# smithlabcode/abismal

Hardware: AMD Instinct MI355X
Metric: mapped reads/sec (whole node), 100 bp SE on hg38-scale index (higher is better)
Workload: dtype u64

## Files before the change

abismal_amd/api.py:

```python
import ctypes as C
import os

import numpy as np

_HERE = os.path.dirname(os.path.abspath(__file__))

SE_T_RICH, SE_A_RICH, SE_RANDOM = 0, 1, 2
PE_NORMAL, PE_PBAT, PE_RANDOM = 0, 1, 2
RECORDS_SAM, RECORDS_BAM = 0, 1

HIT_DTYPE = np.dtype([("diffs", "<i2"), ("flags", "<u2"), ("pos", "<u4")])
PAIR_DTYPE = np.dtype([("aln_score", "<i2"), ("reserved", "<i2"), ("r1", HIT_DTYPE), ("r2", HIT_DTYPE)])

EXPORTED_SYMBOLS = [
    "abm_last_error", "abm_default_params", "abm_index_open", "abm_index_close",
    "abm_index_max_candidates", "abm_index_n_chroms", "abm_index_chrom_name",
    "abm_index_chrom_starts", "abm_index_bytes", "abm_index_build", "abm_index_build_targets", "abm_index_build_opts", "abm_index_window", "abm_ctx_create", "abm_ctx_reserve", "abm_ctx_destroy",
    "abm_map_se_batch", "abm_map_se_batch_sliced", "abm_ctx_slice_results", "abm_map_se_device", "abm_map_pe_batch", "abm_map_pe_device",
    "abm_max_read_length", "abm_ctx_reads_too_long", "abm_ctx_filter_on_planes", "abm_ctx_long_cigars", "abm_ctx_take_work", "abm_ctx_set_phase_stamps", "abm_ctx_set_read_cycles", "abm_ctx_set_timing", "abm_ctx_take_kernel_time", "abm_ctx_take_kernel_times", "abm_ctx_take_work_tiers", "abm_stats_allreduce",
    "abm_device_count", "abm_host_alloc", "abm_host_free", "abm_index_set_seed_extension", "abm_index_set_max_candidates", "abm_index_set_direct_narrowing", "abm_ctx_seed_extension", "abm_ctx_rebuild_seed_extension", "abm_device_numa_node",
    "abm_ctx_set_pe_split", "abm_ctx_pe_split_stats", "abm_ctx_pe_timed_launches", "abm_ctx_set_pair_phases", "abm_device_memory", "abm_ctx_pe_footprint", "abm_index_set_seed_extension_cap", "abm_ctx_pinned_bytes", "abm_ctx_set_sam_tails", "abm_ctx_slice_sam_tails", "abm_ctx_pe_sam_tails", "abm_ctx_set_record_format",
    "abm_index_set_window_records", "abm_ctx_window_records",
]


class AbismalAmdError(RuntimeError):
    pass


class Params(C.Structure):
    _fields_ = [("max_candidates", C.c_uint32), ("valid_frac", C.c_double), ("min_frag", C.c_uint32),
                ("max_frag", C.c_uint32), ("allow_ambig", C.c_int32)]

    def __init__(self, max_candidates=0, valid_frac=0.1, min_frag=32, max_frag=3000, allow_ambig=0):
# ... 44 lines not shown
    lib.abm_ctx_destroy.argtypes = [C.c_void_p]
    lib.abm_ctx_reserve.argtypes = [C.c_void_p, C.c_uint64, C.c_uint32, C.c_int]
    lib.abm_max_read_length.restype = C.c_uint32
    lib.abm_ctx_reads_too_long.argtypes = [C.c_void_p]
    lib.abm_ctx_reads_too_long.restype = C.c_uint64
    lib.abm_ctx_filter_on_planes.argtypes = [C.c_void_p]
    lib.abm_ctx_filter_on_planes.restype = C.c_int
    lib.abm_ctx_take_work.argtypes = [C.c_void_p, C.POINTER(C.c_uint64)]
    lib.abm_ctx_long_cigars.argtypes = [C.c_void_p, C.c_void_p, C.c_uint64, C.POINTER(C.c_uint64)]
    lib.abm_ctx_set_timing.argtypes = [C.c_void_p, C.c_int]
    lib.abm_ctx_set_phase_stamps.argtypes = [C.c_void_p, C.c_int]
    lib.abm_ctx_set_read_cycles.argtypes = [C.c_void_p, C.c_void_p]
    lib.abm_ctx_take_kernel_time.argtypes = [C.c_void_p, C.POINTER(C.c_uint64), C.POINTER(C.c_double)]
    lib.abm_ctx_take_kernel_times.argtypes = [C.c_void_p, C.POINTER(C.c_double), C.c_uint64, C.POINTER(C.c_uint64)]
    lib.abm_ctx_take_work_tiers.argtypes = [C.c_void_p, C.POINTER(C.c_uint64)]
    vp = C.c_void_p
    lib.abm_map_se_batch.argtypes = [vp, C.c_int, C.POINTER(Params), C.c_uint64, vp, vp, vp, vp, C.c_uint64, vp]
    lib.abm_map_se_device.argtypes = [vp, C.c_int, C.POINTER(Params), C.c_uint64, vp, vp, C.c_uint32, vp, vp,
                                      C.c_uint32, vp, vp, vp]
    lib.abm_map_pe_batch.argtypes = [vp, C.c_int, C.POINTER(Params), C.c_uint64, vp, vp, vp, vp, vp, vp, vp,
                                     vp, vp, vp, vp, C.c_uint64]
    lib.abm_map_pe_device.argtypes = [vp, C.c_int, C.POINTER(Params), C.c_uint64, vp, vp, vp, vp, C.c_uint32,
                                      vp, vp, vp, vp, vp, C.c_uint32, vp, vp, vp, vp]
    _lib = lib
    return lib


def _check(rc):
    if rc != 0:
        raise AbismalAmdError(load_library().abm_last_error().decode(errors="replace"))
# ... 257 lines not shown
    def take_work_tiers(self):
        out = (C.c_uint64 * 32)()
        _check(self._lib.abm_ctx_take_work_tiers(self.handle, out))
        keys = ["seed_offsets", "search_probes", "candidates", "index_run_lines", "set_updates", "alignments",
                "cyc_probe_narrow", "cyc_gather_hamming", "cyc_replay", "cyc_se_fallback", "cyc_total",
                "window_cache_hits", "cyc_sort_unique", "cyc_score_pairable", "cyc_mate", "cyc_best_single"]
        return [dict(zip(keys, [int(x) for x in out[16 * t:16 * t + 16]])) for t in range(2)]

    def take_work(self):
        out = (C.c_uint64 * 16)()
        _check(self._lib.abm_ctx_take_work(self.handle, out))
        keys = ["seed_offsets", "search_probes", "candidates", "read_words", "set_updates", "alignments"]
        d = dict(zip(keys, [int(x) for x in out[:6]]))
        d["window_cache_hits"] = int(out[11])
        d["single_job_reads"] = int(out[12])
        if out[10]:
            d["light_filter_steps"], d["fifo_updates"], d["filter_steps"] = int(out[13]), int(out[14]), int(out[15])
        if out[10]:
            d["phase_cycles"] = dict(zip(["probe_narrow", "gather_hamming", "replay", "align", "total"],
                                         [int(x) for x in out[6:11]]))
        return d

    def set_pe_split(self, split=-1, seed_cap=0, hand_entries=0):
        self._lib.abm_ctx_set_pe_split.argtypes = [C.c_void_p, C.c_int, C.c_uint32, C.c_uint64]
        _check(self._lib.abm_ctx_set_pe_split(self.handle, int(split), int(seed_cap), int(hand_entries)))

    def pe_split_stats(self):
        out = (C.c_uint64 * 4)()
        self._lib.abm_ctx_pe_split_stats.argtypes = [C.c_void_p, C.POINTER(C.c_uint64)]
        _check(self._lib.abm_ctx_pe_split_stats(self.handle, out))
# ... 18 lines not shown
```

abismal_amd/csrc/abm_api.hip:

```cpp
#include "../../include/abismal_amd.h"
#include "abm_index_file.hpp"
#include "abm_index_build.hpp"
#include "abm_kernels.hpp"

#include <rccl/rccl.h>

#include <algorithm>
#include <cctype>
#include <chrono>
#include <cstdio>
#include <cstdlib>
#include <cstring>
#include <iterator>
#include <map>
#include <mutex>
#include <stdexcept>
#include <string>
#include <thread>
#include <vector>

namespace {

thread_local std::string g_error;

// ... 342 lines not shown
  a.cig_arena_count = ctx->cig_arena_count.p;
  if (pinned) ctx->h_tail.p[0] = ctx->h_tail.p[1] = 0;
  a.cig_arena = pinned ? ctx->h_arena.p : ctx->cig_arena.p;
  a.cig_arena_cap = static_cast<abm::u32>(std::min<size_t>(pinned ? ctx->h_arena.cap : ctx->cig_arena.cap, 0xFFFFFF00u));
}

abm::u32 se_text_stride(const abm_ctx *ctx, const LaunchShape &s, abm::u32 cig_stride, bool host_results, bool sliced) {
  if (!ctx->sam_on || !host_results || !sliced) return 0;
  if (ctx->sam_format == ABM_RECORDS_BAM && ctx->phase_stamps) return 0;
  const abm::u32 stride = ctx->sam_format == ABM_RECORDS_BAM ? bam_stride_for(s.eff_len, cig_stride) : sam_stride_for(ctx, s.eff_len, cig_stride);
  return stride <= abm::sam_line_room(s.GW, s.tb_extra) ? stride : 0;
}

void se_reserve(abm_ctx *ctx, uint64_t n, const LaunchShape &s, uint32_t n_slices, bool host_results, abm::u32 sam_stride) {
  ctx->packed.reserve(n * 4 * s.W); ctx->lens.reserve(n);
  ctx->work.reserve(32); ctx->next_read.reserve(64);
  if (n < (1ull << 32)) {
    ctx->order.reserve(n); ctx->cls.reserve(n);
    if (n_slices) { ctx->slice_id.reserve(n); ctx->slice_left.reserve(n_slices); ctx->slice_hist.reserve(abm::order_sliced_hist_words(n_slices)); }
    else ctx->class33.reserve(33);
  }
  arena_reserve(ctx, 2 * n, host_results);
  if (sam_stride) { ctx->h_sam.reserve(static_cast<size_t>(n) * sam_stride); ctx->h_sam_len.reserve(n); }
}

void se_long_reads(abm_ctx *ctx, const abm::SeArgs &main, uint64_t n, const char *d_blob, const uint64_t *d_off,
                   abm::u32 max_len, double valid_frac, HostMode host, hipStream_t st) {
  if (n >= (1ull << 32)) throw std::invalid_argument("batch too large for the long-read launch (>= 2^32 reads)");
  ctx->long_list.reserve(n);
  ctx->long_count.reserve(1);
  HIPCHK(hipMemsetAsync(ctx->long_count.p, 0, 4, st));
// ... 264 lines not shown
  PeLaunch t2;
};
PePlan pe_plan(const abm_ctx *ctx, uint64_t n, const LaunchShape &s, abm::u32 cig_stride, bool host_results) {
  PePlan p{};
  p.split = pe_split_on(ctx);
  p.sam_stride = pe_text_stride(ctx, s, cig_stride, host_results);
  p.scap = pe_seed_cap(ctx);
  if (p.split) p.seed = pe_seed_launch(s, n);
  else p.t1 = pe_whole_launch(ctx, s, n, false, p.sam_stride != 0);
  p.t2 = pe_whole_launch(ctx, s, n, true, p.sam_stride != 0);
  return p;
}

void pe_reserve(abm_ctx *ctx, uint64_t n, const LaunchShape &s, abm::u32 mode_slots, bool host_results, const PePlan &p) {
  ctx->packed.reserve(n * 4 * s.W); ctx->packed2.reserve(n * 4 * s.W); ctx->lens.reserve(n); ctx->lens2.reserve(n);
  ctx->work.reserve(32); ctx->next_read.reserve(64);
  ctx->order.reserve(n); ctx->cls.reserve(n); ctx->class33.reserve(33);
  ctx->need_big.reserve(n); ctx->subset.reserve(n); ctx->subset_count.reserve(1);
  if (p.sam_stride) { ctx->h_sam.reserve(static_cast<size_t>(2 * n) * p.sam_stride); ctx->h_sam_len.reserve(2 * n); ctx->h_pe_kind.reserve(n); }
  arena_reserve(ctx, 4 * n, host_results);
  if (!p.split) ctx->payload1.reserve(static_cast<size_t>(std::max(p.t1.waves, 0)) * abm::kPeTier1Cap);
  else {
    const size_t hand_cap = pe_hand_entries(ctx, n), stage = p.scap > abm::kPeTier1Cap ? static_cast<size_t>(p.seed.grid) * p.scap : 0;
    ctx->hand_hdr.reserve(n * mode_slots * 2); ctx->hand_count.reserve(1);
    ctx->hand_pos.reserve(hand_cap); ctx->hand_d.reserve(hand_cap);
    ctx->stage_pos.reserve(stage); ctx->stage_d.reserve(stage);
    ctx->subset_b.reserve(n); ctx->subset_count_b.reserve(1); ctx->class33_b.reserve(33);
  }
  pe_tier2_reserve(ctx, static_cast<size_t>(std::max(p.t2.waves, 0)));
}

// ... 479 lines not shown
          rep.dix.wrec = nullptr;
          rep.dix.wrec_t0 = rep.dix.wrec_a0 = rep.dix.wrec_blocks = rep.dix.wrec_back = rep.dix.wrec_max_len = 0;
          try { build_wrec(rep, *ix); build_ext(rep, *ix, tables_maxc); }
          catch (...) { free_wrec(rep); (void)hipFree(arena); rep.arena = nullptr; throw; }
        }
        ++rep.refs;
        c->holds_replica = true;
        c->rep = &rep;
        c->dix = rep.dix;
        c->kernel_turn = &rep.kernel_turn;
      }
      HIPCHK(hipStreamCreateWithFlags(&c->stream, hipStreamNonBlocking));
      HIPCHK(hipEventCreateWithFlags(&c->last_done, hipEventDisableTiming));
      HIPCHK(hipHostMalloc(reinterpret_cast<void **>(&c->drained), sizeof(abm::u32), hipHostMallocMapped | hipHostMallocCoherent));
      *c->drained = 0;
      c->work.reserve(32);
      HIPCHK(hipMemset(c->work.p, 0, 32 * sizeof(unsigned long long)));
    }
    catch (...) { abm_ctx_destroy(c); throw; }
    *out = c;
  });
}

void abm_ctx_destroy(abm_ctx *c) {
  if (!c) return;
  (void)hipSetDevice(c->device);
  if (c->stream) (void)hipStreamDestroy(c->stream);
  if (c->last_done) (void)hipEventDestroy(c->last_done);
  if (c->drained) (void)hipHostFree(c->drained);
  if (c->holds_replica && c->rep) {
    std::lock_guard<std::mutex> lk(c->rep->mu);
    if (--c->rep->refs == 0) {
// ... 38 lines not shown
    unsigned long long tmp[32];
    HIPCHK(hipMemcpy(tmp, ctx->work.p, sizeof(tmp), hipMemcpyDeviceToHost));
    HIPCHK(hipMemset(ctx->work.p, 0, sizeof(tmp)));
    for (int k = 0; k < 16; ++k) out[k] = tmp[k] + tmp[16 + k];
  });
}

int abm_ctx_take_work_tiers(abm_ctx *ctx, uint64_t out[32]) {
  return guarded([&] {
    HIPCHK(hipSetDevice(ctx->device));
    HIPCHK(hipDeviceSynchronize());
    unsigned long long tmp[32];
    HIPCHK(hipMemcpy(tmp, ctx->work.p, sizeof(tmp), hipMemcpyDeviceToHost));
    HIPCHK(hipMemset(ctx->work.p, 0, sizeof(tmp)));
    for (int k = 0; k < 32; ++k) out[k] = tmp[k];
  });
}

int abm_ctx_set_timing(abm_ctx *ctx, int enable) {
  return guarded([&] {
    if (!ctx) throw std::invalid_argument("ctx is null");
    std::lock_guard<std::mutex> lk(ctx->mu);
    ctx->timing = enable != 0;
  });
}

int abm_ctx_take_kernel_time(abm_ctx *ctx, uint64_t *launches, double *total_ms) {
  return guarded([&] {
    if (!ctx || !launches || !total_ms) throw std::invalid_argument("null argument");
    std::lock_guard<std::mutex> lk(ctx->mu);
// ... 393 lines not shown
    std::vector<abm_hit> hits(m), h2(m);
    std::vector<abm_pair> pairs(m);
    std::vector<uint32_t> cig(m * (L + 2)), cig2(m * (L + 2));
    std::vector<uint64_t> co(m + 1), co2(m + 1);
    abm_params par;
    abm_default_params(&par);
    int rc;
    if (!paired) rc = abm_map_se_batch(ctx, ABM_SE_T_RICH, &par, m, blob.data(), off.data(), hits.data(), cig.data(), cig.size(), co.data());
    else rc = abm_map_pe_batch(ctx, ABM_PE_NORMAL, &par, m, blob.data(), off.data(), blob.data(), off.data(), pairs.data(), hits.data(),
                               h2.data(), cig.data(), co.data(), cig2.data(), co2.data(), cig.size());
    if (rc != 0) throw std::runtime_error(g_error);
    {
      std::lock_guard<std::mutex> lk(ctx->mu);
      HIPCHK(hipSetDevice(ctx->device));
      HIPCHK(hipDeviceSynchronize());
      HIPCHK(hipMemset(ctx->work.p, 0, 32 * sizeof(unsigned long long)));
    }
  });
}

int abm_ctx_long_cigars(abm_ctx *ctx, uint32_t *out_ops, uint64_t capacity, uint64_t *n_ops) {
  return guarded([&] {
    if (!ctx || !n_ops) throw std::invalid_argument("null argument");
    std::lock_guard<std::mutex> lk(ctx->mu);
    HIPCHK(hipSetDevice(ctx->device));
    HIPCHK(hipEventSynchronize(ctx->last_done));
    uint32_t cnt = 0;
    if (ctx->cig_arena_count.p) HIPCHK(hipMemcpy(&cnt, ctx->cig_arena_count.p, 4, hipMemcpyDeviceToHost));
    cnt = static_cast<uint32_t>(std::min<uint64_t>(cnt, ctx->cig_arena.cap));
    *n_ops = cnt;
    if (cnt > capacity) throw std::length_error("capacity too small for the long CIGARs");
// ... 66 lines not shown
```

abismal_amd/csrc/abm_kernels.hip:

```cpp
#include <type_traits>
#include "abm_kernels_core.hpp"
#include "abm_sam.hpp"

#ifndef ABM_SE_WAVES_PER_SIMD
#define ABM_SE_WAVES_PER_SIMD 5
#endif


namespace abm {

__global__ __launch_bounds__(256) void pack_reads_kernel(const char *__restrict__ blob,
                                                         const u64 *__restrict__ off, u64 n_reads,
                                                         u32 W, u64 *__restrict__ packed,
                                                         u32 *__restrict__ lens) {
  const u64 gid = static_cast<u64>(blockIdx.x) * blockDim.x + threadIdx.x;
  const u64 r = gid / W;
  const u32 w = static_cast<u32>(gid % W);
  if (r >= n_reads)
    return;
  const u64 b = off[r];
  const u32 L = static_cast<u32>(off[r + 1] - b);
  if (w == 0)
    lens[r] = L;
  u64 ft = 0, fa = 0, rt = 0, ra = 0;
// ... 118 lines not shown
  lds.hres = reinterpret_cast<u16 *>(lds.lbest);
  lds.G = a.G;
  lds.smark[lane] = 0; lds.smark[64 + lane] = 0;
  u32 seg_epoch = 0;

  const u32 n_calls = a.mode == 2 ? 4u : 2u;
  const u32 call_rc = a.mode == 2 ? 0xCu  : 0x2u ;
  const u32 call_ar = a.mode == 2 ? 0x6u  : (a.mode == 1 ? 0x3u : 0x0u);

  WorkTally wt = {0, 0, 0, 0, 0, 0, 0, 0, 0, 0, 0, 0, 0, 0};
  const CigarSink sink = {a.cig_stride, a.ctmp_cap, a.cig_arena, a.cig_arena_count, a.cig_arena_cap, (!LONG && a.sam_tail) ? lds.jpos : nullptr};
  const u64 n_items = a.n_reads;
  long long t_begin = 0, t_a = 0, t_b = 0;
  ABM_STAMP(t_begin);
  u32 n_aln = 0, n_single = 0;
  bool overflow = false, too_long = false;

  const u64 dealt = gridDim.x;
  auto next_read = [&]() -> u64 {
    unsigned long long v = 0;
    if (lane == 0) {
      v = atomicAdd(a.next_read, 1ull) + dealt;
      if (v >= n_items && a.drained) __hip_atomic_store(a.drained, 1u, __ATOMIC_RELAXED, __HIP_MEMORY_SCOPE_SYSTEM);
    }
    return (static_cast<u64>(static_cast<u32>(uni(static_cast<int>(v >> 32)))) << 32) |
           static_cast<u32>(uni(static_cast<int>(v)));
  };
  u64 r_next = blockIdx.x;
  while (r_next < n_items) {
    const u64 slot = r_next;
// ... 28 lines not shown
      SeSet S;
      S.begin_read(L);
      for (u32 cidx = 0; cidx < n_calls; ++cidx) {
        const bool rc = (call_rc >> cidx) & 1u, ar = (call_ar >> cidx) & 1u;
        const bool g_to_a = rc != ar;
        const u32 enc = (rc ? 2u : 0u) + (g_to_a ? 1u : 0u);
        const u32 flags = (rc ? kFlagRC : 0u) | (ar ? kFlagARich : 0u);
        S.cutoff = S.good_cutoff;
        seed_pass<true, TIMED, COOP, REC>(a.ix, lds, enc, g_to_a, flags, L, S, wt, seg_epoch);
        if (S.sz != static_cast<int>(kSeCap) || S.cutoff > S.good_cutoff) {
          S.cutoff = S.top_d();
          seed_pass<false, TIMED, COOP, REC>(a.ix, lds, enc, g_to_a, flags, L, S, wt, seg_epoch);
        }
      }
      ABM_STAMP(t_a);
      choose_se<LONG>(a.ix, lds, L, a.valid_frac, S, best, cig_out, sink, n_ops, rd_overflow, n_aln, n_single);
      overflow |= rd_overflow;
      ABM_STAMP(t_b);
      if (TIMED) wt.t_align += t_b - t_a;
    }
    if constexpr (!LONG) {
      if (a.sam_tail != nullptr) {
        const u32 len = (L > a.max_len) ? 0xFFFFFFFFu : format_sam_tail<BAM>(a, lds.tb, lds.jpos, r, (L >= a.ix.min_len) ? L : 0u, best, best.pos != 0 ? n_ops : 0u);
        if (lane == 0) store_out(a.sam_len + r, len);
      }
    }
    if (lane == 0) {
      store_out(a.res + r, best);
      store_out(a.cig_n + r, best.pos != 0 ? n_ops : 0u);
      if (TIMED && a.read_cycles) a.read_cycles[r] = static_cast<u32>((clock64() - t_read) >> 10);
    }
// ... 19 lines not shown
      atomicAdd(&a.work[2], static_cast<unsigned long long>(s2));
      atomicAdd(&a.work[3], static_cast<unsigned long long>(s3));
      atomicAdd(&a.work[4], static_cast<unsigned long long>(wt.updates));
      atomicAdd(&a.work[5], static_cast<unsigned long long>(n_aln));
      atomicAdd(&a.work[11], static_cast<unsigned long long>(wsum_hits));
      atomicAdd(&a.work[12], static_cast<unsigned long long>(n_single));
      if (TIMED) {
        atomicAdd(&a.work[6], static_cast<unsigned long long>(wt.t_probe));
        atomicAdd(&a.work[7], static_cast<unsigned long long>(wt.t_stream));
        atomicAdd(&a.work[8], static_cast<unsigned long long>(wt.t_replay));
        atomicAdd(&a.work[9], static_cast<unsigned long long>(wt.t_align));
        atomicAdd(&a.work[10], static_cast<unsigned long long>(phase_stamp() - t_begin));
        atomicAdd(&a.work[13], static_cast<unsigned long long>(wt.light_steps));
        atomicAdd(&a.work[14], static_cast<unsigned long long>(wt.fifo_updates));
        atomicAdd(&a.work[15], static_cast<unsigned long long>(wt.steps));
      }
    }
  }
  if (lane == 0 && (overflow || too_long))
    atomicOr(a.status, (overflow ? 1u : 0u) | (too_long ? 2u : 0u));
  if (a.host_tail != nullptr && lane == 0) {
    __threadfence();
    const u32 before = atomicAdd(a.finished, 1u);
    if (before + 1u == gridDim.x) {
      __threadfence();
      a.host_tail[0] = __hip_atomic_load(a.cig_arena_count, __ATOMIC_RELAXED, __HIP_MEMORY_SCOPE_AGENT);
      a.host_tail[1] = __hip_atomic_load(a.status, __ATOMIC_RELAXED, __HIP_MEMORY_SCOPE_AGENT);
    }
  }
}
// ... 364 lines not shown
```

abismal_amd/csrc/abm_kernels.hpp:

```cpp
#pragma once
#include "abm_device.hpp"

namespace abm {

struct SeArgs {
  DevIndex ix;
  const u64 *packed;
  const u32 *lens;
  const u32 *order;
  u64 n_reads;
  u32 W, WB, GW;
  u32 max_len;
  u32 tb_extra;
  u32 G;
  int mode;
  double valid_frac;
  double size_frac;
  Hit *res;
  u32 *cig;
  u32 cig_stride;
  u32 ctmp_cap;
  u8 *long_tb;
  u32 *long_ctmp;
  u64 long_tb_bytes;
// ... 7 lines not shown
  u32 *finished;
  u32 *host_tail;
  const u16 *slice_id;
  u32 *slice_left;
  u32 *slice_done;
  const char *blob;
  const u64 *off;
  char *sam_tail;
  u32 *sam_len;
  u32 sam_stride;
  int sam_allow_ambig;
  int sam_format;
  u32 *read_cycles;
  unsigned long long *work;
};

struct PeArgs {
  DevIndex ix;
  const u64 *packed1, *packed2;
  const u32 *lens1, *lens2;
  const u32 *order;
  const u32 *subset;
  const u32 *subset_count;
  u64 n_pairs;
  u32 W, WB, GW, tb_extra, G, max_len;
  int mode;
  double valid_frac;
  u32 min_frag, max_frag;
  int allow_ambig;
  Hit *pairs;
// ... 105 lines not shown
```

abismal_amd/csrc/abm_kernels_core.hpp:

```cpp
#pragma once
#include "abm_kernels.hpp"

namespace abm {

struct SeSet {
  static constexpr bool kFifo = true;
  static constexpr bool kAppend = false;
  int hk;
  u32 pf;
  u32 pp;
  int sz, cutoff, good_cutoff;
  int best_d;
  u32 best_f, best_p;
  bool sure_ambig;

  __device__ __forceinline__ static int key_d(int k) { return k >> 8; }
  __device__ __forceinline__ void begin_read(u32 readlen) {
    const int worst = static_cast<i16>(0.4 * readlen);
    hk = worst * 256; pf = 0; pp = 0;
    sz = 1;
    cutoff = worst;
    good_cutoff = static_cast<i16>(readlen / 10u);
    best_d = worst; best_f = 0; best_p = 0;
    sure_ambig = false;
// ... 1060 lines not shown
    cur = valid ? c : 0;
    if (valid && c > bestv) { bestv = c; bestrow = i; }
    if (TB && assigned) lds.tb[i * bw + jl] = static_cast<u8>(valid ? (arrow | (c > 0 ? 4 : 0)) : 3);
  }
}

struct CigarSink {
  u32 stride;
  u32 ctmp_cap;
  u32 *arena;
  u32 *arena_count;
  u32 arena_cap;
  u32 *fin;
};

__device__ __forceinline__ void wave_cigar(const u8 *tb, u32 *ctmp, int L, int diffs, int max_diffs,
                                           int score, int best_r, int best_c, u32 *cig_out,
                                           const CigarSink &sink, u32 &n_ops, int &ins, int &del, u32 &aln_len,
                                           u32 &t_pos, bool &overflow) {
  const int lane = lane_id();
  ins = del = 0;
  if (score == 0 || diffs == 0) {
    if (lane == 0) { store_out(cig_out, static_cast<u32>(L) << 4); if (sink.fin) sink.fin[0] = static_cast<u32>(L) << 4; }
    n_ops = 1;
    aln_len = static_cast<u32>(L);
    return;
  }
  const int bw = band_for(diffs, max_diffs);
  int r = best_r, c = best_c;
  const int clip_tail = (L + (bw - 1)) - (r + c);
  u32 n = 0;
  auto emit = [&](u32 run, int op) {
    if (n < sink.ctmp_cap) { if (lane == 0) ctmp[n] = (run << 4) | static_cast<u32>(op); }
    const int r8 = static_cast<int>(static_cast<u8>(run));
    ins = op == 1 ? static_cast<i16>(ins + r8) : ins;
    del = op == 2 ? static_cast<i16>(del + r8) : del;
    ++n;
  };
  auto step = [&](int a) {
    if (a != 1) --r;
    if (a == 1) --c;
    if (a == 2) ++c;
  };
  int op = uni(tb[r * bw + c]) & 3;
  step(op);
  u32 run = 1;
  for (;;) {
    const int cell = uni(tb[r * bw + c]);
    if (!(cell & 4)) break;
    const int a = cell & 3;
    step(a);
    if (a != op) { emit(run, op); run = 0; }
    ++run;
    op = a;
  }
  emit(run, op);
  const int clip_head = (r + c) - (bw - 1);
  wave_sync();
  const u32 full = n + (clip_head > 0) + (clip_tail > 0);
  u32 *dst = cig_out;
  u32 body = n, total = full;
  if (full > sink.stride) {
    u32 at = 0xFFFFFFFFu;
    if (sink.arena != nullptr && n <= sink.ctmp_cap) {
      if (lane == 0) at = atomicAdd(sink.arena_count, full);
      at = static_cast<u32>(uni(static_cast<int>(at)));
      if (at > sink.arena_cap || full > sink.arena_cap - at) at = 0xFFFFFFFFu;
    }
    if (at != 0xFFFFFFFFu) {
      dst = sink.arena + at;
      if (lane == 0) store_out(cig_out, at);
    }
    else {
// ... 1 lines not shown
      body = min(min(n, sink.ctmp_cap), sink.stride);
      total = min(body + (clip_head > 0) + (clip_tail > 0), sink.stride);
    }
  }
  for (u32 k = lane; k < total; k += 64) {
    u32 v;
    const u32 kk = k - (clip_head > 0 ? 1u : 0u);
    if (clip_head > 0 && k == 0) v = (static_cast<u32>(clip_head) << 4) | 4u;
    else if (kk < body) v = ctmp[body - 1 - kk];
    else v = (static_cast<u32>(clip_tail) << 4) | 4u;
    store_out(dst + k, v);
    if (sink.fin && k < kSeCap) sink.fin[k] = v;
  }
  n_ops = full;
  aln_len = static_cast<u32>(L - clip_tail - clip_head);
  t_pos = t_pos - static_cast<u32>((bw - 1) / 2) + static_cast<u32>(r);
}

__device__ __forceinline__ int edit_distance(int scr, u32 len, int ins, int del) {
  if (scr == 0)
    return static_cast<i16>(len);
  const int A = static_cast<i16>(scr + 4 * (ins + del));
  const u32 num = 2u * (len - static_cast<u32>(ins)) - static_cast<u32>(A);
  const int mism = static_cast<i16>(num / 5u);
  return static_cast<i16>(mism + ins + del);
}

__device__ __forceinline__ bool long_enough(u32 aln_len, u32 readlen, u32 kMinReadLen) {
  const double min_frac = 1.0 - 0.4;
  return aln_len >= max(kMinReadLen, static_cast<u32>(min_frac * readlen));
}
// ... 154 lines not shown
}

struct QuadJob {
  u32 mv, ma, ml;
  int qoff_lo, qoff_hi;
  int g_lo, g_hi;
  int gs_lo, gs_hi;
};

typedef unsigned short u16x2 __attribute__((ext_vector_type(2)));
__device__ __forceinline__ int wave_min_i32(int x) {
#pragma unroll
  for (int d = 32; d >= 1; d >>= 1) x = min(x, __shfl_xor(x, d));
  return x;
}
__device__ __forceinline__ void wavefront_quad(const WaveLds &lds, const QuadJob &jp, const QuadJob &jq, int dp, int dq,
                                               int o, int width, int L, int w_min, int w_max, u32 &bestp, u32 &bestq) {
  const int t_start = max(0, w_min - 1), t_end = 2 * (L - 1 + w_max) + 1;
  const int n_total = (t_end - t_start) / 2 + 1;
  const int W = static_cast<int>(lds.W), GW = static_cast<int>(lds.GW);
  const int q0p = ((t_start - dp - o) >> 1) + o - width, q0q = ((t_start + 1 - dq - o) >> 1) + o - width;
  const bool in_slot = width != 0;
  const int q_lo = wave_min_i32(in_slot ? min(q0p, q0q) : 0x3fffffff), q_hi = wave_max_i32(in_slot ? max(q0p, q0q) : -0x3fffffff);
  const int n_mid0 = min(max(1 - q_lo, 0), n_total), n_mid1 = min(max(L - 1 - q_hi, n_mid0), n_total);
  u32 curp = 0, curq = 0, pub = 0, Mp = 0, Mq = 0;
  bestp = bestq = 0;
  auto refill = [&](const QuadJob &j, int q) -> u32 {
    const int i0 = q - o + width;
    u64 lo = 0, hi = 0;
    if (j.mv & 0xFFFFu) lo = nibbles16(lds.qpk + j.qoff_lo, W, q) & nibbles16(lds.gwin + j.g_lo * GW, GW, j.gs_lo + i0 - 1);
    if (j.mv >> 16) hi = nibbles16(lds.qpk + j.qoff_hi, W, q) & nibbles16(lds.gwin + j.g_hi * GW, GW, j.gs_hi + i0 - 1);
    lo |= lo >> 1; lo |= lo >> 2;
    hi |= hi >> 1; hi |= hi >> 2;
    return every_fourth_bit(lo) | (every_fourth_bit(hi) << 16);
  };
  auto step_delta = [&](u32 &M) -> u32 {
    const u16x2 bits = __builtin_bit_cast(u16x2, M & 0x00010001u);
    M >>= 1;
    const u16x2 five = {5, 5}, minus3 = {0xFFFD, 0xFFFD};
    return __builtin_bit_cast(u32, static_cast<u16x2>(bits * five + minus3));
  };
  auto fast = [&](const QuadJob &j, u32 &cur, u32 &M, u32 &best) {
    const u32 lf = static_cast<u32>(from_prev_lane(static_cast<int>(pub))), up = static_cast<u32>(from_next_lane(static_cast<int>(pub)));
    u32 c = pk_max(pk_add(cur, step_delta(M)), 0u);
    c = pk_max(c, pk_add(up, 0xFFFCFFFCu) & j.ma);
    c = pk_max(c, pk_add(lf, 0xFFFCFFFCu) & j.ml);
    cur = c & j.mv;
    best = pk_max(best, cur);
    pub = cur;
  };
  auto slow = [&](const QuadJob &j, int q, u32 &cur, u32 &M, u32 &best) {
    const u32 lf = static_cast<u32>(from_prev_lane(static_cast<int>(pub))), up = static_cast<u32>(from_next_lane(static_cast<int>(pub)));
    u32 c = pk_max(pk_add(cur, step_delta(M)), 0u);
    c = pk_max(c, pk_add(up, 0xFFFCFFFCu) & (q < L - 1 ? j.ma : 0u));
    c = pk_max(c, pk_add(lf, 0xFFFCFFFCu) & (q > 0 ? j.ml : 0u));
    cur = static_cast<u32>(q) < static_cast<u32>(L) ? (c & j.mv) : 0u;
    best = pk_max(best, cur);
    pub = cur;
  };
  int n = 0;
#pragma clang loop unroll(disable)
  for (int seg = 0; seg < 3; ++seg) {
    const int end = seg == 0 ? n_mid0 : (seg == 1 ? n_mid1 : n_total);
    while (n < end) {
      if ((n & 15) == 0) { Mp = refill(jp, n + q0p); Mq = refill(jq, n + q0q); }
      const int stop = min(end, (n | 15) + 1);
      if (seg == 1) {
        for (; n < stop; ++n) { fast(jp, curp, Mp, bestp); fast(jq, curq, Mq, bestq); }
      }
      else {
        for (; n < stop; ++n) { slow(jp, n + q0p, curp, Mp, bestp); slow(jq, n + q0q, curq, Mq, bestq); }
      }
    }
  }
}

__device__ __forceinline__ int score_round_quad(const DevIndex &ix, const WaveLds &lds, int first, int n_jobs, int L, int md,
                                                int qbase) {
  const int lane = lane_id();
  QuadJob ja = {0, 0, 0, 0, 0, 0, 0, 0, 0}, jb = {0, 0, 0, 0, 0, 0, 0, 0, 0};
  int used = 0, s = first, w_min = 64, w_max = 0, my_o = 0, my_w = 0;
  while (s < n_jobs) {
    const int cnt = min(4, n_jobs - s);
    if (s - first + cnt > static_cast<int>(lds.max_jobs)) break;
    int bwh[4], width = 0;
#pragma unroll
    for (int h = 0; h < 4; ++h) {
      bwh[h] = h < cnt ? band_for(static_cast<int>(lds.jdf[s + h]) >> 16, md) : 0;
      width = max(width, bwh[h]);
    }
    if (used + width > 64) break;
    const int o = lane - used, K = (width - 1) / 2, c = o - K;
    const bool in = o >= 0 && o < width;
// ... 14 lines not shown
        const int gs = static_cast<int>(t_beg & 15u) - (K - k);
        if (h >> 1) { j.qoff_hi = qoff; j.g_hi = s + h - first; j.gs_hi = gs; }
        else { j.qoff_lo = qoff; j.g_lo = s + h - first; j.gs_lo = gs; }
      }
    }
    used += width;
    w_min = min(w_min, width);
    w_max = max(w_max, width);
    s += cnt;
  }
  stage_windows(ix, lds, first, s - first, md);
  wave_sync();
  const int t_start = max(0, w_min - 1);
  const bool even = ((t_start - my_o) & 1) == 0;
  u32 bp, bq;
  wavefront_quad(lds, even ? ja : jb, even ? jb : ja, even ? 0 : 1, even ? 1 : 0, my_o, my_w, L, w_min, w_max, bp, bq);
  const u32 best_a = even ? bp : bq, best_b = even ? bq : bp;
  int base = 0, mine = 0;
  for (int k = first; k < s;) {
    const int cnt = min(4, s - k);
    int width = 0;
#pragma unroll
    for (int h = 0; h < 4; ++h)
      if (h < cnt) width = max(width, band_for(static_cast<int>(lds.jdf[k + h]) >> 16, md));
    const bool in = lane >= base && lane < base + width;
    const u32 xa = wave_max_pk(in ? best_a : 0u), xb = cnt > 1 ? wave_max_pk(in ? best_b : 0u) : 0u;
    if (lane == k - first) mine = static_cast<int>(xa & 0xFFFFu);
    if (lane == k + 1 - first && cnt > 1) mine = static_cast<int>(xb & 0xFFFFu);
    if (lane == k + 2 - first && cnt > 2) mine = static_cast<int>(xa >> 16);
    if (lane == k + 3 - first && cnt > 3) mine = static_cast<int>(xb >> 16);
    base += width;
// ... 5 lines not shown
  return s;
}

#ifndef ABM_QUAD_MIN_JOBS
#define ABM_QUAD_MIN_JOBS 1
#endif
constexpr int kQuadMinJobs = ABM_QUAD_MIN_JOBS;
template <bool WRAP = false>
__device__ __forceinline__ int score_jobs(const DevIndex &ix, const WaveLds &lds, int first, int n_jobs, int L, int md, int qbase) {
  if constexpr (!WRAP) {
    if (n_jobs - first >= kQuadMinJobs) return score_round_quad(ix, lds, first, n_jobs, L, md, qbase);
  }
  return score_round<WRAP>(ix, lds, first, n_jobs, L, md, qbase);
}

template <bool WRAP = false>
__device__ __forceinline__ void choose_se(const DevIndex &ix, const WaveLds &lds, u32 L, double frac,
                                          SeSet &S, Hit &best, u32 *cig_out, const CigarSink &sink,
                                          u32 &n_ops, bool &overflow, u32 &n_aln, u32 &n_single) {
  const int lane = lane_id();
  const int Ls = static_cast<i16>(L);
  const int md = static_cast<i16>(frac * static_cast<u32>(Ls));
  const int perfect = static_cast<i16>(2 * L);
  n_ops = 0;
  if (S.best_p != 0) {
    best.diffs = static_cast<i16>(S.best_d); best.flags = static_cast<u16>(S.best_f); best.pos = S.best_p;
    if (lane == 0) { store_out(cig_out, L << 4); if (sink.fin) sink.fin[0] = L << 4; }
    n_ops = 1;
    return;
  }
  const bool mine = lane < S.sz;
  const int slot_of = S.hk & 255;
  const u32 e_pos = __shfl(S.pp, slot_of), e_flags = __shfl(S.pf, slot_of);
  const int e_d = SeSet::key_d(S.hk);
// ... 77 lines not shown
    if (sc <= 0) { best.flags = static_cast<u16>(kFlagAmbig); return; }
  }
  u32 alen = 0, pos = b_pos;
  int n_ins = 0, n_del = 0;
  wave_cigar(lds.tb, lds.ctmp, static_cast<int>(L), b_diffs, md, sc, br, bc, cig_out, sink, n_ops,
             n_ins, n_del, alen, pos, overflow);
  wave_sync();
  const int nm = edit_distance(top, alen, n_ins, n_del);
  if (long_enough(alen, static_cast<u32>(Ls), ix.min_len) && nm <= md) {
    best.diffs = static_cast<i16>(nm);
    best.pos = pos;
  }
}


}
```

include/abismal_amd.h:

```cpp
#ifndef ABISMAL_AMD_H
#define ABISMAL_AMD_H

#include <stddef.h>
#include <stdint.h>

#ifdef __cplusplus
extern "C" {
#endif

typedef struct abm_index abm_index;
typedef struct abm_ctx abm_ctx;

typedef struct { int16_t diffs; uint16_t flags; uint32_t pos; } abm_hit;

typedef struct { int16_t aln_score; int16_t reserved; abm_hit r1, r2; } abm_pair;

typedef struct {
  uint32_t max_candidates;
  double valid_frac;
  uint32_t min_frag;
  uint32_t max_frag;
  int32_t allow_ambig;
} abm_params;

// ... 81 lines not shown
int abm_ctx_long_cigars(abm_ctx *ctx, uint32_t *out_ops, uint64_t capacity, uint64_t *n_ops);

enum {
  ABM_STATUS_CIGAR_OVERFLOW = 1u,
  ABM_STATUS_READ_TOO_LONG = 2u,
  ABM_STATUS_SET_OVERFLOW = 4u
};
uint32_t abm_max_read_length(void);
uint64_t abm_ctx_reads_too_long(abm_ctx *ctx);

int abm_ctx_filter_on_planes(const abm_ctx *ctx);

int abm_ctx_take_work(abm_ctx *ctx, uint64_t out[16]);
int abm_ctx_set_phase_stamps(abm_ctx *ctx, int enable);
int abm_ctx_take_work_tiers(abm_ctx *ctx, uint64_t out[32]);
int abm_ctx_set_read_cycles(abm_ctx *ctx, uint32_t *d_read_cycles);
int abm_ctx_set_pair_phases(abm_ctx *ctx, uint32_t *d_pair_phases);

int abm_ctx_set_timing(abm_ctx *ctx, int enable);
int abm_ctx_take_kernel_time(abm_ctx *ctx, uint64_t *launches, double *total_ms);
int abm_ctx_take_kernel_times(abm_ctx *ctx, double *ms_out, uint64_t capacity, uint64_t *launches);

int abm_stats_allreduce(abm_ctx *const *ctxs, int n_ctx, uint64_t *const *counters);

#ifdef __cplusplus
}
#endif
#endif
```

Before: 22.62 million.

## Score best-diff pilot candidate first and prune remaining wavefronts below its score

For short-read SE mapping, the candidate with the fewest seed diffs is aligned and traced first. Its score then becomes a floor that lets the packed quad wavefront stop early once no lane can reach it, using an upper bound of match score times remaining read bases. If another candidate wins, the traceback is redone for that candidate. The cost is an extra alignment pass in that case, added per-16-step ballot checks, and new iteration counters exposed through the work buffer.

```diff
diff --git a/abismal_amd/api.py b/abismal_amd/api.py
--- a/abismal_amd/api.py
+++ b/abismal_amd/api.py
@@ -17,7 +17,7 @@
     "abm_index_max_candidates", "abm_index_n_chroms", "abm_index_chrom_name",
     "abm_index_chrom_starts", "abm_index_bytes", "abm_index_build", "abm_index_build_targets", "abm_index_build_opts", "abm_index_window", "abm_ctx_create", "abm_ctx_reserve", "abm_ctx_destroy",
     "abm_map_se_batch", "abm_map_se_batch_sliced", "abm_ctx_slice_results", "abm_map_se_device", "abm_map_pe_batch", "abm_map_pe_device",
-    "abm_max_read_length", "abm_ctx_reads_too_long", "abm_ctx_filter_on_planes", "abm_ctx_long_cigars", "abm_ctx_take_work", "abm_ctx_set_phase_stamps", "abm_ctx_set_read_cycles", "abm_ctx_set_timing", "abm_ctx_take_kernel_time", "abm_ctx_take_kernel_times", "abm_ctx_take_work_tiers", "abm_stats_allreduce",
+    "abm_max_read_length", "abm_ctx_reads_too_long", "abm_ctx_filter_on_planes", "abm_ctx_long_cigars", "abm_ctx_take_work", "abm_ctx_set_phase_stamps", "abm_ctx_set_read_cycles", "abm_ctx_set_timing", "abm_ctx_take_kernel_time", "abm_ctx_take_kernel_times", "abm_ctx_take_work_tiers", "abm_ctx_take_score_iterations", "abm_stats_allreduce",
     "abm_device_count", "abm_host_alloc", "abm_host_free", "abm_index_set_seed_extension", "abm_index_set_max_candidates", "abm_index_set_direct_narrowing", "abm_ctx_seed_extension", "abm_ctx_rebuild_seed_extension", "abm_device_numa_node",
     "abm_ctx_set_pe_split", "abm_ctx_pe_split_stats", "abm_ctx_pe_timed_launches", "abm_ctx_set_pair_phases", "abm_device_memory", "abm_ctx_pe_footprint", "abm_index_set_seed_extension_cap", "abm_ctx_pinned_bytes", "abm_ctx_set_sam_tails", "abm_ctx_slice_sam_tails", "abm_ctx_pe_sam_tails", "abm_ctx_set_record_format",
     "abm_index_set_window_records", "abm_ctx_window_records",
@@ -92,6 +92,8 @@
     lib.abm_ctx_take_kernel_time.argtypes = [C.c_void_p, C.POINTER(C.c_uint64), C.POINTER(C.c_double)]
     lib.abm_ctx_take_kernel_times.argtypes = [C.c_void_p, C.POINTER(C.c_double), C.c_uint64, C.POINTER(C.c_uint64)]
     lib.abm_ctx_take_work_tiers.argtypes = [C.c_void_p, C.POINTER(C.c_uint64)]
+    if hasattr(lib, "abm_ctx_take_score_iterations"):
+        lib.abm_ctx_take_score_iterations.argtypes = [C.c_void_p, C.POINTER(C.c_uint64)]
     vp = C.c_void_p
     lib.abm_map_se_batch.argtypes = [vp, C.c_int, C.POINTER(Params), C.c_uint64, vp, vp, vp, vp, C.c_uint64, vp]
     lib.abm_map_se_device.argtypes = [vp, C.c_int, C.POINTER(Params), C.c_uint64, vp, vp, C.c_uint32, vp, vp,
@@ -379,6 +381,10 @@
         d = dict(zip(keys, [int(x) for x in out[:6]]))
         d["window_cache_hits"] = int(out[11])
         d["single_job_reads"] = int(out[12])
+        if out[10] and hasattr(self._lib, "abm_ctx_take_score_iterations"):
+            it = (C.c_uint64 * 2)()
+            _check(self._lib.abm_ctx_take_score_iterations(self.handle, it))
+            d["score_iterations"], d["score_iterations_full"] = int(it[0]), int(it[1])
         if out[10]:
             d["light_filter_steps"], d["fifo_updates"], d["filter_steps"] = int(out[13]), int(out[14]), int(out[15])
         if out[10]:
diff --git a/abismal_amd/csrc/abm_api.hip b/abismal_amd/csrc/abm_api.hip
--- a/abismal_amd/csrc/abm_api.hip
+++ b/abismal_amd/csrc/abm_api.hip
@@ -380,7 +380,7 @@
 
 void se_reserve(abm_ctx *ctx, uint64_t n, const LaunchShape &s, uint32_t n_slices, bool host_results, abm::u32 sam_stride) {
   ctx->packed.reserve(n * 4 * s.W); ctx->lens.reserve(n);
-  ctx->work.reserve(32); ctx->next_read.reserve(64);
+  ctx->work.reserve(abm::kWorkWords); ctx->next_read.reserve(64);
   if (n < (1ull << 32)) {
     ctx->order.reserve(n); ctx->cls.reserve(n);
     if (n_slices) { ctx->slice_id.reserve(n); ctx->slice_left.reserve(n_slices); ctx->slice_hist.reserve(abm::order_sliced_hist_words(n_slices)); }
@@ -675,7 +675,7 @@
 
 void pe_reserve(abm_ctx *ctx, uint64_t n, const LaunchShape &s, abm::u32 mode_slots, bool host_results, const PePlan &p) {
   ctx->packed.reserve(n * 4 * s.W); ctx->packed2.reserve(n * 4 * s.W); ctx->lens.reserve(n); ctx->lens2.reserve(n);
-  ctx->work.reserve(32); ctx->next_read.reserve(64);
+  ctx->work.reserve(abm::kWorkWords); ctx->next_read.reserve(64);
   ctx->order.reserve(n); ctx->cls.reserve(n); ctx->class33.reserve(33);
   ctx->need_big.reserve(n); ctx->subset.reserve(n); ctx->subset_count.reserve(1);
   if (p.sam_stride) { ctx->h_sam.reserve(static_cast<size_t>(2 * n) * p.sam_stride); ctx->h_sam_len.reserve(2 * n); ctx->h_pe_kind.reserve(n); }
@@ -1185,8 +1185,8 @@
       HIPCHK(hipEventCreateWithFlags(&c->last_done, hipEventDisableTiming));
       HIPCHK(hipHostMalloc(reinterpret_cast<void **>(&c->drained), sizeof(abm::u32), hipHostMallocMapped | hipHostMallocCoherent));
       *c->drained = 0;
-      c->work.reserve(32);
-      HIPCHK(hipMemset(c->work.p, 0, 32 * sizeof(unsigned long long)));
+      c->work.reserve(abm::kWorkWords);
+      HIPCHK(hipMemset(c->work.p, 0, abm::kWorkWords * sizeof(unsigned long long)));
     }
     catch (...) { abm_ctx_destroy(c); throw; }
     *out = c;
@@ -1255,6 +1255,18 @@
     HIPCHK(hipMemcpy(tmp, ctx->work.p, sizeof(tmp), hipMemcpyDeviceToHost));
     HIPCHK(hipMemset(ctx->work.p, 0, sizeof(tmp)));
     for (int k = 0; k < 32; ++k) out[k] = tmp[k];
+  });
+}
+
+int abm_ctx_take_score_iterations(abm_ctx *ctx, uint64_t out[2]) {
+  return guarded([&] {
+    if (!ctx) throw std::invalid_argument("ctx is null");
+    HIPCHK(hipSetDevice(ctx->device));
+    HIPCHK(hipDeviceSynchronize());
+    unsigned long long tmp[2];
+    HIPCHK(hipMemcpy(tmp, ctx->work.p + abm::kWorkScoreIters, sizeof(tmp), hipMemcpyDeviceToHost));
+    HIPCHK(hipMemset(ctx->work.p + abm::kWorkScoreIters, 0, sizeof(tmp)));
+    out[0] = tmp[0]; out[1] = tmp[1];
   });
 }
 
@@ -1678,7 +1690,7 @@
       std::lock_guard<std::mutex> lk(ctx->mu);
       HIPCHK(hipSetDevice(ctx->device));
       HIPCHK(hipDeviceSynchronize());
-      HIPCHK(hipMemset(ctx->work.p, 0, 32 * sizeof(unsigned long long)));
+      HIPCHK(hipMemset(ctx->work.p, 0, abm::kWorkWords * sizeof(unsigned long long)));
     }
   });
 }
diff --git a/abismal_amd/csrc/abm_kernels.hip b/abismal_amd/csrc/abm_kernels.hip
--- a/abismal_amd/csrc/abm_kernels.hip
+++ b/abismal_amd/csrc/abm_kernels.hip
@@ -156,6 +156,7 @@
   long long t_begin = 0, t_a = 0, t_b = 0;
   ABM_STAMP(t_begin);
   u32 n_aln = 0, n_single = 0;
+  u32 score_iters[2] = {0, 0};
   bool overflow = false, too_long = false;
 
   const u64 dealt = gridDim.x;
@@ -214,7 +215,7 @@
         }
       }
       ABM_STAMP(t_a);
-      choose_se<LONG>(a.ix, lds, L, a.valid_frac, S, best, cig_out, sink, n_ops, rd_overflow, n_aln, n_single);
+      choose_se<LONG, !LONG, TIMED>(a.ix, lds, L, a.valid_frac, S, best, cig_out, sink, n_ops, rd_overflow, n_aln, n_single, score_iters);
       overflow |= rd_overflow;
       ABM_STAMP(t_b);
       if (TIMED) wt.t_align += t_b - t_a;
@@ -264,6 +265,8 @@
         atomicAdd(&a.work[13], static_cast<unsigned long long>(wt.light_steps));
         atomicAdd(&a.work[14], static_cast<unsigned long long>(wt.fifo_updates));
         atomicAdd(&a.work[15], static_cast<unsigned long long>(wt.steps));
+        atomicAdd(&a.work[kWorkScoreIters], static_cast<unsigned long long>(score_iters[0]));
+        atomicAdd(&a.work[kWorkScoreIters + 1], static_cast<unsigned long long>(score_iters[1]));
       }
     }
   }
diff --git a/abismal_amd/csrc/abm_kernels.hpp b/abismal_amd/csrc/abm_kernels.hpp
--- a/abismal_amd/csrc/abm_kernels.hpp
+++ b/abismal_amd/csrc/abm_kernels.hpp
@@ -45,6 +45,7 @@
   u32 *read_cycles;
   unsigned long long *work;
 };
+constexpr u32 kWorkScoreIters = 32, kWorkWords = 34;
 
 struct PeArgs {
   DevIndex ix;
diff --git a/abismal_amd/csrc/abm_kernels_core.hpp b/abismal_amd/csrc/abm_kernels_core.hpp
--- a/abismal_amd/csrc/abm_kernels_core.hpp
+++ b/abismal_amd/csrc/abm_kernels_core.hpp
@@ -1098,24 +1098,20 @@
   u32 *fin;
 };
 
-__device__ __forceinline__ void wave_cigar(const u8 *tb, u32 *ctmp, int L, int diffs, int max_diffs,
-                                           int score, int best_r, int best_c, u32 *cig_out,
-                                           const CigarSink &sink, u32 &n_ops, int &ins, int &del, u32 &aln_len,
-                                           u32 &t_pos, bool &overflow) {
+struct CigarWalk {
+  u32 n;
+  int clip_head, clip_tail;
+  int r;
+};
+__device__ __forceinline__ CigarWalk cigar_walk(const u8 *tb, u32 *ctmp, u32 ctmp_cap, int L, int bw, int best_r, int best_c,
+                                                int &ins, int &del) {
   const int lane = lane_id();
   ins = del = 0;
-  if (score == 0 || diffs == 0) {
-    if (lane == 0) { store_out(cig_out, static_cast<u32>(L) << 4); if (sink.fin) sink.fin[0] = static_cast<u32>(L) << 4; }
-    n_ops = 1;
-    aln_len = static_cast<u32>(L);
-    return;
-  }
-  const int bw = band_for(diffs, max_diffs);
   int r = best_r, c = best_c;
   const int clip_tail = (L + (bw - 1)) - (r + c);
   u32 n = 0;
   auto emit = [&](u32 run, int op) {
-    if (n < sink.ctmp_cap) { if (lane == 0) ctmp[n] = (run << 4) | static_cast<u32>(op); }
+    if (n < ctmp_cap) { if (lane == 0) ctmp[n] = (run << 4) | static_cast<u32>(op); }
     const int r8 = static_cast<int>(static_cast<u8>(run));
     ins = op == 1 ? static_cast<i16>(ins + r8) : ins;
     del = op == 2 ? static_cast<i16>(del + r8) : del;
@@ -1141,6 +1137,13 @@
   emit(run, op);
   const int clip_head = (r + c) - (bw - 1);
   wave_sync();
+  return {n, clip_head, clip_tail, r};
+}
+__device__ __forceinline__ void cigar_publish(const u32 *ctmp, const CigarWalk &w, int L, int bw, u32 *cig_out,
+                                              const CigarSink &sink, u32 &n_ops, u32 &aln_len, u32 &t_pos, bool &overflow) {
+  const int lane = lane_id();
+  const u32 n = w.n;
+  const int clip_head = w.clip_head, clip_tail = w.clip_tail;
   const u32 full = n + (clip_head > 0) + (clip_tail > 0);
   u32 *dst = cig_out;
   u32 body = n, total = full;
@@ -1172,7 +1175,22 @@
   }
   n_ops = full;
   aln_len = static_cast<u32>(L - clip_tail - clip_head);
-  t_pos = t_pos - static_cast<u32>((bw - 1) / 2) + static_cast<u32>(r);
+  t_pos = t_pos - static_cast<u32>((bw - 1) / 2) + static_cast<u32>(w.r);
+}
+__device__ __forceinline__ void wave_cigar(const u8 *tb, u32 *ctmp, int L, int diffs, int max_diffs,
+                                           int score, int best_r, int best_c, u32 *cig_out,
+                                           const CigarSink &sink, u32 &n_ops, int &ins, int &del, u32 &aln_len,
+                                           u32 &t_pos, bool &overflow) {
+  if (score == 0 || diffs == 0) {
+    ins = del = 0;
+    if (lane_id() == 0) { store_out(cig_out, static_cast<u32>(L) << 4); if (sink.fin) sink.fin[0] = static_cast<u32>(L) << 4; }
+    n_ops = 1;
+    aln_len = static_cast<u32>(L);
+    return;
+  }
+  const int bw = band_for(diffs, max_diffs);
+  const CigarWalk w = cigar_walk(tb, ctmp, sink.ctmp_cap, L, bw, best_r, best_c, ins, del);
+  cigar_publish(ctmp, w, L, bw, cig_out, sink, n_ops, aln_len, t_pos, overflow);
 }
 
 __device__ __forceinline__ int edit_distance(int scr, u32 len, int ins, int del) {
@@ -1357,8 +1375,13 @@
   for (int d = 32; d >= 1; d >>= 1) x = min(x, __shfl_xor(x, d));
   return x;
 }
+constexpr int kScoreMatch = 2, kScoreMismatch = -3, kScoreIndel = -4;
+static_assert(kScoreMatch > 0 && kScoreMismatch <= kScoreMatch && kScoreIndel <= 0,
+              "the floor's bound: no step gains more than kScoreMatch per read base, and none that consumes no read base gains");
+template <bool FLOOR = false>
 __device__ __forceinline__ void wavefront_quad(const WaveLds &lds, const QuadJob &jp, const QuadJob &jq, int dp, int dq,
-                                               int o, int width, int L, int w_min, int w_max, u32 &bestp, u32 &bestq) {
+                                               int o, int width, int L, int w_min, int w_max, u32 &bestp, u32 &bestq,
+                                               int floor = 0, int *iters = nullptr) {
   const int t_start = max(0, w_min - 1), t_end = 2 * (L - 1 + w_max) + 1;
   const int n_total = (t_end - t_start) / 2 + 1;
   const int W = static_cast<int>(lds.W), GW = static_cast<int>(lds.GW);
@@ -1377,17 +1400,25 @@
     hi |= hi >> 1; hi |= hi >> 2;
     return every_fourth_bit(lo) | (every_fourth_bit(hi) << 16);
   };
+  constexpr unsigned short kStep = kScoreMatch - kScoreMismatch, kMiss = static_cast<unsigned short>(kScoreMismatch);
+  constexpr u32 kGap = static_cast<u32>(static_cast<unsigned short>(kScoreIndel)) * 0x00010001u;
+  static_assert(kStep == 5 && kMiss == 0xFFFD && kGap == 0xFFFCFFFCu, "the packed cell's constants");
   auto step_delta = [&](u32 &M) -> u32 {
     const u16x2 bits = __builtin_bit_cast(u16x2, M & 0x00010001u);
     M >>= 1;
-    const u16x2 five = {5, 5}, minus3 = {0xFFFD, 0xFFFD};
+    const u16x2 five = {kStep, kStep}, minus3 = {kMiss, kMiss};
     return __builtin_bit_cast(u32, static_cast<u16x2>(bits * five + minus3));
+  };
+  auto alive = [&](const QuadJob &j, u32 cur, u32 best, int q_done) -> bool {
+    const int left = min(max(L - 1 - q_done, 0), L);
+    const u32 ub = pk_max(best, pk_add(cur, static_cast<u32>(kScoreMatch * left) * 0x00010001u));
+    return ((j.mv & 0xFFFFu) && static_cast<int>(ub & 0xFFFFu) >= floor) || ((j.mv >> 16) && static_cast<int>(ub >> 16) >= floor);
   };
   auto fast = [&](const QuadJob &j, u32 &cur, u32 &M, u32 &best) {
     const u32 lf = static_cast<u32>(from_prev_lane(static_cast<int>(pub))), up = static_cast<u32>(from_next_lane(static_cast<int>(pub)));
     u32 c = pk_max(pk_add(cur, step_delta(M)), 0u);
-    c = pk_max(c, pk_add(up, 0xFFFCFFFCu) & j.ma);
-    c = pk_max(c, pk_add(lf, 0xFFFCFFFCu) & j.ml);
+    c = pk_max(c, pk_add(up, kGap) & j.ma);
+    c = pk_max(c, pk_add(lf, kGap) & j.ml);
     cur = c & j.mv;
     best = pk_max(best, cur);
     pub = cur;
@@ -1395,8 +1426,8 @@
   auto slow = [&](const QuadJob &j, int q, u32 &cur, u32 &M, u32 &best) {
     const u32 lf = static_cast<u32>(from_prev_lane(static_cast<int>(pub))), up = static_cast<u32>(from_next_lane(static_cast<int>(pub)));
     u32 c = pk_max(pk_add(cur, step_delta(M)), 0u);
-    c = pk_max(c, pk_add(up, 0xFFFCFFFCu) & (q < L - 1 ? j.ma : 0u));
-    c = pk_max(c, pk_add(lf, 0xFFFCFFFCu) & (q > 0 ? j.ml : 0u));
+    c = pk_max(c, pk_add(up, kGap) & (q < L - 1 ? j.ma : 0u));
+    c = pk_max(c, pk_add(lf, kGap) & (q > 0 ? j.ml : 0u));
     cur = static_cast<u32>(q) < static_cast<u32>(L) ? (c & j.mv) : 0u;
     best = pk_max(best, cur);
     pub = cur;
@@ -1406,7 +1437,12 @@
   for (int seg = 0; seg < 3; ++seg) {
     const int end = seg == 0 ? n_mid0 : (seg == 1 ? n_mid1 : n_total);
     while (n < end) {
-      if ((n & 15) == 0) { Mp = refill(jp, n + q0p); Mq = refill(jq, n + q0q); }
+      if ((n & 15) == 0) {
+        if constexpr (FLOOR) {
+          if (n != 0 && !__any(alive(jp, curp, bestp, n - 1 + q0p) || alive(jq, curq, bestq, n - 1 + q0q))) { *iters = n; return; }
+        }
+        Mp = refill(jp, n + q0p); Mq = refill(jq, n + q0q);
+      }
       const int stop = min(end, (n | 15) + 1);
       if (seg == 1) {
         for (; n < stop; ++n) { fast(jp, curp, Mp, bestp); fast(jq, curq, Mq, bestq); }
@@ -1416,10 +1452,15 @@
       }
     }
   }
-}
-
+  if constexpr (FLOOR) *iters = n_total;
+}
+__device__ __forceinline__ int quad_iterations(int L, int w_min, int w_max) {
+  return (2 * (L - 1 + w_max) + 1 - max(0, w_min - 1)) / 2 + 1;
+}
+
+template <bool FLOOR = false>
 __device__ __forceinline__ int score_round_quad(const DevIndex &ix, const WaveLds &lds, int first, int n_jobs, int L, int md,
-                                                int qbase) {
+                                                int qbase, int floor = 0, u32 *iters = nullptr) {
   const int lane = lane_id();
   QuadJob ja = {0, 0, 0, 0, 0, 0, 0, 0, 0}, jb = {0, 0, 0, 0, 0, 0, 0, 0, 0};
   int used = 0, s = first, w_min = 64, w_max = 0, my_o = 0, my_w = 0;
@@ -1464,7 +1505,13 @@
   const int t_start = max(0, w_min - 1);
   const bool even = ((t_start - my_o) & 1) == 0;
   u32 bp, bq;
-  wavefront_quad(lds, even ? ja : jb, even ? jb : ja, even ? 0 : 1, even ? 1 : 0, my_o, my_w, L, w_min, w_max, bp, bq);
+  if constexpr (FLOOR) {
+    int ran = 0;
+    wavefront_quad<true>(lds, even ? ja : jb, even ? jb : ja, even ? 0 : 1, even ? 1 : 0, my_o, my_w, L, w_min, w_max, bp, bq, floor, &ran);
+    iters[0] += static_cast<u32>(ran);
+    iters[1] += static_cast<u32>(quad_iterations(L, w_min, w_max));
+  }
+  else wavefront_quad(lds, even ? ja : jb, even ? jb : ja, even ? 0 : 1, even ? 1 : 0, my_o, my_w, L, w_min, w_max, bp, bq);
   const u32 best_a = even ? bp : bq, best_b = even ? bq : bp;
   int base = 0, mine = 0;
   for (int k = first; k < s;) {
@@ -1500,10 +1547,60 @@
   return score_round<WRAP>(ix, lds, first, n_jobs, L, md, qbase);
 }
 
-template <bool WRAP = false>
+__device__ __forceinline__ int list_se_jobs(const WaveLds &lds, const SeSet &S, int Ls) {
+  const int lane = lane_id();
+  const bool mine = lane < S.sz;
+  const int slot_of = S.hk & 255;
+  const u32 e_pos = __shfl(S.pp, slot_of), e_flags = __shfl(S.pf, slot_of);
+  const int e_d = SeSet::key_d(S.hk);
+  const u64 key = (static_cast<u64>(e_pos) << 16) | e_flags;
+  bool dup = false;
+  for (int k = 0; k < S.sz; ++k) {
+    const u64 kk = rdlane(key, k);
+    dup |= (mine && k < lane && kk == key);
+  }
+  const int invalid_at = static_cast<i16>(0.4 * Ls);
+  const bool is_job = mine && !dup && e_pos != 0 && e_d < invalid_at;
+  const u64 jobs = __ballot(is_job);
+  int rank = 0;
+  for (int k = 0; k < S.sz; ++k) {
+    const u64 kk = rdlane(key, k);
+    rank += ((jobs >> k) & 1) && kk < key;
+  }
+  const int n_jobs = __popcll(jobs);
+  if (is_job) {
+    lds.jpos[rank] = e_pos;
+    lds.jdf[rank] = (static_cast<u32>(e_d) << 16) | e_flags;
+  }
+  wave_sync();
+  return n_jobs;
+}
+
+__device__ __forceinline__ void first_maximum(int bw, int bv, int brow, int &sc, int &br, int &bc) {
+  const int lane = lane_id();
+  const u64 k64 = (static_cast<u64>(static_cast<u32>(bv)) << 32) |
+                  (static_cast<u64>(0xFFFFu - static_cast<u32>(brow)) << 8) |
+                  static_cast<u64>(0xFFu - static_cast<u32>(lane));
+  const u64 topk = wave_max_u64(lane < bw ? k64 : 0ull);
+  br = static_cast<int>(0xFFFFu - static_cast<u32>((topk >> 8) & 0xFFFFu));
+  bc = static_cast<int>(0xFFu - static_cast<u32>(topk & 0xFFu));
+  sc = static_cast<i16>(static_cast<int>(topk >> 32));
+}
+
+template <bool TALLY>
+__device__ __forceinline__ void choose_se_pilot(const DevIndex &ix, const WaveLds &lds, u32 L, double frac, SeSet &S, Hit &best,
+                                                u32 *cig_out, const CigarSink &sink, u32 &n_ops, bool &overflow, u32 &n_aln,
+                                                u32 &n_single, u32 *iters);
+
+template <bool WRAP = false, bool PILOT = false, bool TALLY = false>
 __device__ __forceinline__ void choose_se(const DevIndex &ix, const WaveLds &lds, u32 L, double frac,
                                           SeSet &S, Hit &best, u32 *cig_out, const CigarSink &sink,
-                                          u32 &n_ops, bool &overflow, u32 &n_aln, u32 &n_single) {
+                                          u32 &n_ops, bool &overflow, u32 &n_aln, u32 &n_single, u32 *iters = nullptr) {
+  if constexpr (PILOT) {
+    static_assert(!WRAP && kTracebackByRows && kQuadMinJobs <= 1, "the pilot order: 32-bit scores, every round on the packed cells");
+    choose_se_pilot<TALLY>(ix, lds, L, frac, S, best, cig_out, sink, n_ops, overflow, n_aln, n_single, iters);
+    return;
+  }
   const int lane = lane_id();
   const int Ls = static_cast<i16>(L);
   const int md = static_cast<i16>(frac * static_cast<u32>(Ls));
@@ -1611,4 +1708,105 @@
 }
 
 
-}
+template <bool TALLY>
+__device__ __forceinline__ void choose_se_pilot(const DevIndex &ix, const WaveLds &lds, u32 L, double frac, SeSet &S, Hit &best,
+                                                u32 *cig_out, const CigarSink &sink, u32 &n_ops, bool &overflow, u32 &n_aln,
+                                                u32 &n_single, u32 *iters) {
+  const int lane = lane_id();
+  const int Ls = static_cast<i16>(L);
+  const int md = static_cast<i16>(frac * static_cast<u32>(Ls));
+  const int perfect = static_cast<i16>(2 * L);
+  n_ops = 0;
+  if (S.best_p != 0) {
+    best.diffs = static_cast<i16>(S.best_d); best.flags = static_cast<u16>(S.best_f); best.pos = S.best_p;
+    if (lane == 0) { store_out(cig_out, L << 4); if (sink.fin) sink.fin[0] = L << 4; }
+    n_ops = 1;
+    return;
+  }
+  const int n_jobs = list_se_jobs(lds, S, Ls);
+  best.diffs = 0x7fff; best.flags = 0; best.pos = 0;
+  if (n_jobs == 0) return;
+  const bool single = n_jobs == 1;
+  int pilot = 0;
+  if (!single) pilot = wave_min_i32(lane < n_jobs ? static_cast<int>(((lds.jdf[lane] >> 16) << 8) | static_cast<u32>(lane)) : 0x7fffffff) & 255;
+  const u32 p_pos = lds.jpos[pilot], p_df = lds.jdf[pilot];
+  int trace = pilot;
+  int top = 0, b_diffs = static_cast<int>(p_df) >> 16;
+  u32 b_pos = p_pos, b_flags = p_df & 0xFFFFu;
+  for (bool pilot_pass = !single;; pilot_pass = false) {
+    const int bw = band_for(b_diffs, md);
+    AlnJob job = {0, 0, 0, 0, 0};
+    const u64 t_beg = static_cast<u64>(b_pos) - static_cast<u64>((bw - 1) / 2);
+    if (lane < bw) {
+      job.bw = bw;
+      job.jl = lane;
+      job.qoff = static_cast<int>(enc_of(b_flags) * lds.W);
+      job.t0nib = static_cast<int>(t_beg & 15u);
+    }
+    stage_windows(ix, lds, trace, 1, md);
+    wave_sync();
+    int bv, brow, sc, br, bc;
+    wavefront_rows<true>(lds, job, static_cast<int>(L), bw, bv, brow);
+    first_maximum(bw, bv, brow, sc, br, bc);
+    wave_sync();
+    CigarWalk walk = {0, 0, 0, 0};
+    int n_ins = 0, n_del = 0;
+    if (sc > 0) walk = cigar_walk(lds.tb, lds.ctmp, sink.ctmp_cap, static_cast<int>(L), bw, br, bc, n_ins, n_del);
+    if (single) {
+      ++n_aln;
+      ++n_single;
+      top = sc;
+      if (sc <= 0) { best.flags = static_cast<u16>(kFlagAmbig); return; }
+      best.flags = static_cast<u16>(b_flags);
+    }
+    if (pilot_pass) {
+      u32 mv_pos = 0, mv_df = 0;
+      const bool moves = lane > pilot && lane < n_jobs;
+      if (moves) { mv_pos = lds.jpos[lane]; mv_df = lds.jdf[lane]; }
+      wave_sync();
+      if (moves) { lds.jpos[lane - 1] = mv_pos; lds.jdf[lane - 1] = mv_df; }
+      wave_sync();
+      const int n_rest = n_jobs - 1;
+      int floor = sc, b_at = -1;
+      u32 top_pos = 0;
+      top = 0; b_pos = 0; b_flags = 0; b_diffs = 0x7fff;
+      auto select = [&](int at, u32 pos, u32 df, int s) {
+        const u32 flags = df & 0xFFFFu;
+        ++n_aln;
+        if (s > top) { b_diffs = static_cast<int>(df) >> 16; b_flags = flags; b_pos = pos; top = s; top_pos = pos; b_at = at; }
+        else if (s == top) {
+          const u32 gap = pos > top_pos ? pos - top_pos : top_pos - pos;
+          if (s == perfect ? pos != top_pos : gap > 3u) b_flags |= kFlagAmbig;
+        }
+      };
+      u32 it[2] = {0, 0};
+      for (int s = 0; s < n_rest;) {
+        const int first = s;
+        s = score_round_quad<true>(ix, lds, first, n_rest, static_cast<int>(L), md, 0, floor, it);
+        for (int k = first; k < s; ++k) {
+          if (k == pilot) select(-1, p_pos, p_df, sc);
+          const int sk = static_cast<i16>(lds.lbest[k - first]);
+          select(k, lds.jpos[k], lds.jdf[k], sk);
+          floor = max(floor, sk);
+        }
+        wave_sync();
+      }
+      if (pilot == n_rest) select(-1, p_pos, p_df, sc);
+      if (TALLY) { iters[0] += it[0]; iters[1] += it[1]; }
+      best.flags = static_cast<u16>(b_flags);
+      if (b_pos == 0) return;
+      if (b_at >= 0) { trace = b_at; continue; }
+    }
+    u32 alen = 0, pos = b_pos;
+    cigar_publish(lds.ctmp, walk, static_cast<int>(L), bw, cig_out, sink, n_ops, alen, pos, overflow);
+    wave_sync();
+    const int nm = edit_distance(top, alen, n_ins, n_del);
+    if (long_enough(alen, static_cast<u32>(Ls), ix.min_len) && nm <= md) {
+      best.diffs = static_cast<i16>(nm);
+      best.pos = pos;
+    }
+    return;
+  }
+}
+
+}
diff --git a/include/abismal_amd.h b/include/abismal_amd.h
--- a/include/abismal_amd.h
+++ b/include/abismal_amd.h
@@ -119,6 +119,7 @@
 int abm_ctx_take_work(abm_ctx *ctx, uint64_t out[16]);
 int abm_ctx_set_phase_stamps(abm_ctx *ctx, int enable);
 int abm_ctx_take_work_tiers(abm_ctx *ctx, uint64_t out[32]);
+int abm_ctx_take_score_iterations(abm_ctx *ctx, uint64_t out[2]);
 int abm_ctx_set_read_cycles(abm_ctx *ctx, uint32_t *d_read_cycles);
 int abm_ctx_set_pair_phases(abm_ctx *ctx, uint32_t *d_pair_phases);
 
```

Result: faster. 23.09 million, median of 6 (+2.1%).
